# RagnarGrootKoerkamp/astar-pairwise-aligner

Hardware: AMD Instinct MI355X
Metric: DP cell-updates/sec (GCUPS), full bit-parallel DP, 100kbp@5% div (higher is better)
Workload: dtype u32

## Files before the change

astar-pairwise-aligner_amd/csrc/pa_hip.hip:

```cpp
#include "pa_batch.hpp"
#include "engine_capi.hpp"
#include "trace_kernel.hpp"

#include <algorithm>
#include <chrono>
#include <cmath>
#include <cstdio>
#include <cstdlib>
#include <cstring>
#include <memory>
#include <atomic>
#include <mutex>
#include <thread>
#include <string>
#include <vector>

namespace pa {

enum : uint32_t { kTextFailed = 0xFFFFFFFFu };
__global__ __launch_bounds__(64) void format_pack_kernel(const uint32_t* __restrict__ elems, const uint64_t* __restrict__ off,
                                                         const uint32_t* __restrict__ len, const int32_t* __restrict__ list,
                                                         uint8_t* __restrict__ packed, unsigned long long* __restrict__ total,
                                                         uint32_t* __restrict__ tlen, uint64_t* __restrict__ dst) {
    const int pair = list[blockIdx.x];
// ... 674 lines not shown

static pa_batch* batch_create(const BatchInput& in, bool trace, float band_hint = -1.f, int dt_max_g = 0, int dt_fr_drop = 0,
                              const pa_astarpa2_params* astar = nullptr, int window_override = -1) {
    if (!ensure_device()) return nullptr;
    PhaseClock clock("pa_batch_create");
    auto p = std::make_unique<pa_batch>();
    p->pairs = in.pairs;
    p->trace = trace;
    p->dt_max_g = dt_max_g;
    p->dt_fr_drop = dt_fr_drop;
    CreateRun cr{p.get(), in, astar};
    choose_shape(cr, band_hint, window_override);
    if (!layout_pairs(cr) || (trace && !alloc_trace_buffers(cr)) || !alloc_batch_buffers(cr)) return nullptr;
    clock.mark("host layout + hipMalloc");
    if (!(p->stream = bstream_take()) || !hip_ok(hipEventCreate(&p->ev0), "event") ||
        !hip_ok(hipEventCreate(&p->ev1), "event") || !hip_ok(hipEventCreate(&p->ev2), "event"))
        return nullptr;
    clock.mark("stream + events");
    if (!upload_sequences(cr)) return nullptr;
    clock.mark("upload of the sequences");
    std::vector<int32_t> first;
    plan_strip_jobs(cr, first);
    if (!upload_first_and_desc(cr, first)) return nullptr;
    if (trace && in.pairs) {
        std::vector<TraceJob> tjobs(in.pairs);
        std::vector<uint64_t> src_off(in.pairs);
        if (!make_trace_jobs(cr, tjobs, src_off) || !plan_chunks(cr) || !upload_trace_jobs(cr, tjobs, src_off)) return nullptr;
    }
    apply_pacing(p.get());
    if (!attach_wavelog(p.get())) return nullptr;
    clock.mark("jobs + descriptors");
    if (cr.slice_rows) {
        p->sequential = false;
        p->sliced = slice::create(p->n.data(), p->m.data(), in.pairs, p->code_off.data(), p->prof_off.data(), cr.slice_rows);
        if (!p->sliced) return nullptr;
        clock.mark("bit-sliced plan");
    }
    if (!p->d_jobs.alloc(p->jobs.size() * sizeof(StripJob))) return nullptr;
    if (!p->jobs.empty() &&
        !hip_ok(hipMemcpyAsync(p->d_jobs.ptr, p->jobs.data(), p->jobs.size() * sizeof(StripJob), hipMemcpyHostToDevice, p->stream), "H2D jobs"))
        return nullptr;
    if (!hip_ok(hipStreamSynchronize(p->stream), "sync")) return nullptr;
    return p.release();
}

extern "C" pa_batch* pa_batch_create(const uint8_t* const* a, const size_t* a_len, const uint8_t* const* b,
                                     const size_t* b_len, size_t pairs) {
    return batch_create({a, a_len, b, b_len, pairs}, false);
}

extern "C" pa_batch* pa_batch_create_banded(const uint8_t* const* a, const size_t* a_len, const uint8_t* const* b,
                                            const size_t* b_len, size_t pairs, float divergence_hint) {
    if (!(divergence_hint >= 0.f)) {
        set_error("pa_batch_create_banded: divergence_hint must be >= 0");
        return nullptr;
    }
    return batch_create({a, a_len, b, b_len, pairs}, false, divergence_hint);
}

extern "C" pa_batch* pa_batch_create_trace(const uint8_t* const* a, const size_t* a_len, const uint8_t* const* b,
                                           const size_t* b_len, size_t pairs) {
    return batch_create({a, a_len, b, b_len, pairs}, true);
}

extern "C" pa_batch* pa_batch_create_trace_params(const uint8_t* const* a, const size_t* a_len, const uint8_t* const* b,
                                                  const size_t* b_len, size_t pairs, const pa_astarpa2_params* trace_params) {
    if (!trace_params) return batch_create({a, a_len, b, b_len, pairs}, true);
// ... 200 lines not shown
        set_error(timeout_msg, misc[err_word]);
        return PA_E_TIMEOUT;
    }
    return 0;
}

static void dump_wavelog(const pa_batch* p) {
    std::vector<uint32_t> log(p->jobs.size() * 8);
    if (hip_ok(hipMemcpy(log.data(), p->d_wavelog.ptr, log.size() * 4, hipMemcpyDeviceToHost), "D2H wavelog")) {
        if (FILE* f = std::fopen(getenv("PA_STRIP_WAVELOG"), "w")) {
            std::fprintf(f, "job k word0 xcc se cu simd wave t0 t1 polled\n");
            for (size_t j = 0; j < p->jobs.size(); ++j) {
                const uint32_t* r = &log[8 * j];
                const uint32_t hw = r[0];
                std::fprintf(f, "%zu %d %d %u %u %u %u %u %llu %llu %u\n", j, p->sequential ? p->jobs[j].k : p->k, p->jobs[j].word0, r[1] & 15u,
                             (hw >> 13) & 7u, (hw >> 8) & 15u, (hw >> 4) & 3u, hw & 15u, (unsigned long long)(r[2] | ((uint64_t)r[3] << 32)),
                             (unsigned long long)(r[4] | ((uint64_t)r[5] << 32)), r[6]);
            }
            std::fclose(f);
        }
    }
}

extern "C" int pa_batch_run(pa_batch* p, int32_t* cost_out, float* kernel_ms) {
    if (!p) return PA_E_ARG;
    if (p->astar) {
        float fwd = 0.f;
        const int rc = pa_batch_align(p, cost_out, nullptr, &fwd, nullptr);
        if (kernel_ms) *kernel_ms = fwd;
        return rc;
    }
    hipStream_t s = p->stream;
    if (p->sliced) {
        if (const int rc = batch_forward(p, false)) return rc;
        if (const int rc = slice::run(p->sliced, s, p->d_codes.as<uint32_t>(), p->d_prof.as<uint64_t>(), p->d_sums.as<int32_t>(), p->d_misc.as<uint32_t>() + 4,
                                      p->ev0, p->ev1))
            return rc;
        if (const int rc = read_sums_and_errors(p, cost_out, 5, "device spin timeout in the bit-sliced kernel (err=%u)")) return rc;
        if (kernel_ms && !hip_ok(hipEventElapsedTime(kernel_ms, p->ev0, p->ev1), "elapsed")) return PA_E_HIP;
        for (size_t i = 0; i < p->pairs; ++i)
            if (p->n[i] == 0 || p->m[i] == 0) cost_out[i] = (int32_t)(p->n[i] + p->m[i]);
        return 0;
    }
    if (const int rc = batch_forward(p)) return rc;
    std::vector<int32_t> sums(p->pairs, 0);
    if (const int rc = read_sums_and_errors(p, sums.data(), 1, "device spin timeout (err=%u)")) return rc;
    p->gran_dirty = p->banded && !p->sequential;
    if (p->d_wavelog.ptr) dump_wavelog(p);
    if (kernel_ms) {
        *kernel_ms = 0.f;
        if (!p->jobs.empty() && !hip_ok(hipEventElapsedTime(kernel_ms, p->ev0, p->ev1), "elapsed")) return PA_E_HIP;
    }
    if (p->banded) return banded_finish(p, sums, cost_out, kernel_ms);
    for (size_t i = 0; i < p->pairs; ++i) {
        const size_t n = p->n[i], m = p->m[i], w = (m + 63) / 64;
        if (n == 0) { cost_out[i] = (int32_t)m; continue; }
        if (w == 0) { cost_out[i] = (int32_t)n; continue; }
        cost_out[i] = (int32_t)(w * 64) + sums[i];
    }
    return 0;
}

static pa_astarpa2_params traced_batch_params() {
    engine::AstarPa2Params p = engine::AstarPa2Params::nw();
    p.front.sparse = true;
    p.front.dt_trace = false;
    p.front.incremental_doubling = false;
    pa_astarpa2_params c;
    engine::params_to_c(p, &c);
    return c;
}
// ... 541 lines not shown
```

astar-pairwise-aligner_amd/csrc/pa_hip_internal.hpp:

```cpp
#pragma once
#include <hip/hip_runtime.h>

#include <cstddef>
#include <cstdint>
#include <string>
#include <vector>

#include "../../include/pa_astarpa2.h"
#include "../../include/pa_bitpacking_hip.h"
#include "strip_kernel.hpp"

namespace pa {

constexpr int kWordsPerStrip = 32;

void set_error(const char* fmt, ...);
bool hip_ok(hipError_t e, const char* what);
bool ensure_device();
int device_cus();
int fail(int rc, const char* fmt, ...) __attribute__((format(printf, 2, 3)));

void* pinned_take(size_t bytes, size_t* got);
void pinned_give(void* ptr, size_t size);
hipStream_t stream_take();
// ... 64 lines not shown
    int fill_stride = 0, fill_word0 = 0;
    bool pingpong = false;
    int k = 1;
    uint32_t* ckpt = nullptr;
    int ckpt_stride = 0;
};

void plan_rect(std::vector<StripJob>& jobs, const RectPlan& r);
struct StripPlan {
    int full = 0, tail1 = 0;
    int strips() const { return full + tail1; }
};
StripPlan strip_plan(int w, int k, bool sequential);
size_t rect_granules(int n, int w, int k = 1, bool pingpong = false);
bool launch_strips(const StripJob* d_jobs, int njobs, bool fill, uint32_t* d_ticket_err, hipStream_t s, bool zero_ticket = true,
                   bool scatter = false, int k = 1, int block_waves = kStripBlockWaves, bool ckpt = false);
bool launch_pairs(const StripJob* d_jobs, const int32_t* d_first, int npairs, uint32_t* d_ticket_err, hipStream_t s, int k, bool ckpt = false);
int align_hip(const uint8_t* a, size_t a_len, const uint8_t* b, size_t b_len, const pa_astarpa2_params& params, bool trace, bool self_check,
              int32_t* cost_out, std::string* cigar_out, pa_astarpa2_stats* stats_out);
bool combine_eligible(size_t a_len, size_t b_len, const pa_astarpa2_params& params);
struct CombineInside {
    CombineInside();
    ~CombineInside();
    CombineInside(const CombineInside&) = delete;
    CombineInside& operator=(const CombineInside&) = delete;
};
int combine_align(const uint8_t* a, size_t a_len, const uint8_t* b, size_t b_len, const pa_astarpa2_params& params, int32_t* cost_out,
                  std::string* cigar_out, pa_astarpa2_stats* stats_out);
int search_profile(const uint8_t* pattern, size_t plen, float unmatched_cost, std::vector<uint64_t>& prof, std::vector<uint64_t>& v0);
bool encode_a_device(const uint8_t* d_a, int n, uint32_t* d_codes, uint32_t* d_bad, hipStream_t s);
bool build_b_device(const uint8_t* d_b, int m, uint64_t* d_prof, uint32_t* d_bad, hipStream_t s);
bool encode_pair_device(const uint8_t* d_a, int n, uint32_t* d_codes, int code_words, const uint8_t* d_b, int m, uint64_t* d_prof, uint32_t* bad,
                        hipStream_t s);
struct PairDesc {
    unsigned long long a_off, b_off, code_off, prof_off;
    int n, m;
};
bool encode_batch_device(const uint8_t* d_a_cat, size_t max_n, uint32_t* d_codes_cat, const uint8_t* d_b_cat, size_t max_m, uint64_t* d_prof_cat,
                         const PairDesc* d_desc, size_t pairs, uint32_t* d_bad, hipStream_t s);
unsigned host_threads();
size_t window_words(size_t n, size_t m, bool gcsh, int override_);

}
```

astar-pairwise-aligner_amd/csrc/rect_unit.hip:

```cpp
#include "pa_hip_internal.hpp"

#include <algorithm>
#include <cstdlib>
#include <cstring>
#include <mutex>
#include <set>
#include <utility>
#include <vector>

namespace pa {


__device__ __forceinline__ int rank_acgt(uint8_t c) {
    return c == 'A' ? 0 : c == 'C' ? 1 : c == 'G' ? 2 : c == 'T' ? 3 : -1;
}

__global__ void encode_a_kernel(const uint8_t* __restrict__ a, int n, uint32_t* __restrict__ codes, int nwords,
                                uint32_t* __restrict__ bad) {
    const int i = blockIdx.x * blockDim.x + threadIdx.x;
    if (i >= nwords) return;
    uint32_t w = 0;
    bool invalid = false;
    for (int k = 0; k < 16; ++k) {
        const int c = i * 16 + k;
        if (c < n) {
            const int r = rank_acgt(a[c]);
            invalid |= r < 0;
            w |= (uint32_t)(r & 3) << (2 * k);
        }
    }
    codes[i] = w;
    if (invalid) atomicOr(bad, 1u);
}

__global__ void build_b_kernel(const uint8_t* __restrict__ b, int m, uint64_t* __restrict__ prof, int nwords,
                               uint32_t* __restrict__ bad) {
    const int word = blockIdx.x * (blockDim.x >> 6) + (threadIdx.x >> 6);
    if (word >= nwords) return;
    const int lane = threadIdx.x & 63;
    const int j = word * 64 + lane;
    int r = 3;
    bool invalid = false;
    if (j < m) {
        r = rank_acgt(b[j]);
        invalid = r < 0;
        r &= 3;
    }
    const uint64_t nb0 = __ballot(((r & 1) ^ 1) != 0);
// ... 451 lines not shown
```

astar-pairwise-aligner_amd/csrc/slice_kernel.hpp:

```cpp
#pragma once
#include <hip/hip_runtime.h>
#include <stdint.h>

namespace pa {
namespace slice {

#ifndef PA_SLICE_CLOCK_TURNS
#define PA_SLICE_CLOCK_TURNS 15
#endif
#ifndef PA_SLICE_YIELD
#define PA_SLICE_YIELD 2
#endif
constexpr int kPad = 64;
constexpr int kErrSpin = 7;
constexpr uint32_t kSpinLimit = 1u << 22;

struct SliceGroup {
    uint64_t a_off;
    uint64_t b_off;
    uint64_t h_off;
    uint32_t h_stride;
    int32_t n;
    int32_t nstrips;
    int32_t npairs;
    uint32_t first_pos;
    uint32_t ev_first, ev_count;
    uint32_t pad_;
};
struct SliceEvent {
    int32_t col;
    uint32_t mask;
};
struct SliceJob {
    uint32_t group, strip;
};
struct SlicePair {
    uint64_t code_off, prof_off;
    int32_t n, m;
    uint32_t pair;
    uint32_t pad_;
};

typedef uint32_t pa_slice_u32x2 __attribute__((ext_vector_type(2)));
__device__ __forceinline__ uint32_t dpp_wave_shr1(uint32_t old_, uint32_t src) {
    return (uint32_t)__builtin_amdgcn_update_dpp((int)old_, (int)src, 0x138, 0xf, 0xf, false);
}
__device__ __forceinline__ uint32_t dpp_wave_rol1(uint32_t x) {
    return (uint32_t)__builtin_amdgcn_update_dpp((int)x, (int)x, 0x134, 0xf, 0xf, false);
}
__device__ __forceinline__ uint2 ld_boundary(const uint2* p) {
    const unsigned long long v = __hip_atomic_load((const unsigned long long*)p, __ATOMIC_RELAXED, __HIP_MEMORY_SCOPE_AGENT);
    return make_uint2((uint32_t)v, (uint32_t)(v >> 32));
}
__device__ __forceinline__ void st_boundary(uint2* p, uint32_t hp, uint32_t hm) {
    __hip_atomic_store((unsigned long long*)p, (unsigned long long)hp | ((unsigned long long)hm << 32), __ATOMIC_RELAXED, __HIP_MEMORY_SCOPE_AGENT);
}

#define PA_SLICE_ROW_PAIR(vpA, vmA, vpB, vmB, nb0A, nb1A, nb0B, nb1B, a0, a1, hpp, hmp, hpo, hmo)                                      \
    do {                                                                                                                                \
        uint32_t zA_, zB_, hmA_, hpA_;                                                                                                  \
        asm volatile(                                                                                                                   \
            "v_xor_b32 %[zA], %[a1_], %[nb1A_]\n\t"                                                                                     \
            "v_xor_b32 %[zB], %[a1_], %[nb1B_]\n\t"                                                                                     \
            "v_bitop3_b32 %[zA], %[a0_], %[nb0A_], %[zA] bitop3:0x28\n\t"                                                               \
            "v_bitop3_b32 %[zB], %[a0_], %[nb0B_], %[zB] bitop3:0x28\n\t"                                                               \
            "v_bitop3_b32 %[zA], %[zA], %[vmA_], %[hmp_] bitop3:0xfe\n\t"                                                               \
            "v_and_b32 %[hmA], %[zA], %[vpA_]\n\t"                                                                                      \
            "v_bitop3_b32 %[hpA], %[vmA_], %[zA], %[vpA_] bitop3:0xf1\n\t"                                                              \
            "v_bitop3_b32 %[zB], %[zB], %[vmB_], %[hmA] bitop3:0xfe\n\t"                                                                \
            "v_bitop3_b32 %[vpA_], %[hmp_], %[zA], %[hpp_] bitop3:0xf1\n\t"                                                             \
            "v_and_b32 %[hmB], %[zB], %[vpB_]\n\t"                                                                                      \
            "v_and_b32 %[vmA_], %[hpp_], %[zA]\n\t"                                                                                     \
            "v_bitop3_b32 %[hpB], %[vmB_], %[zB], %[vpB_] bitop3:0xf1\n\t"                                                              \
            "v_bitop3_b32 %[vpB_], %[hmA], %[zB], %[hpA] bitop3:0xf1\n\t"                                                               \
            "v_and_b32 %[vmB_], %[hpA], %[zB]"                                                                                          \
            : [zA] "=&v"(zA_), [zB] "=&v"(zB_), [hmA] "=&v"(hmA_), [hpA] "=&v"(hpA_), [hmB] "=&v"(hmo), [hpB] "=&v"(hpo),              \
              [vpA_] "+v"(vpA), [vmA_] "+v"(vmA), [vpB_] "+v"(vpB), [vmB_] "+v"(vmB)                                                    \
            : [a0_] "v"(a0), [a1_] "v"(a1), [nb0A_] "v"(nb0A), [nb1A_] "v"(nb1A), [nb0B_] "v"(nb0B), [nb1B_] "v"(nb1B), [hpp_] "v"(hpp), \
              [hmp_] "v"(hmp));                                                                                                         \
    } while (0)

#define PA_SLICE_FEED(a0, a1, hpp, hmp, ohp, ohm, cAx, cAy, cHx, cHy)                                                                    \
    asm volatile(                                                                                                                       \
        "s_mov_b64 vcc, 1\n\t"                                                                                                          \
        "v_cndmask_b32_dpp %[a0_], %[a0_], %[cAx_], vcc wave_shr:1 row_mask:0xf bank_mask:0xf bound_ctrl:0\n\t"                         \
        "v_cndmask_b32_dpp %[a1_], %[a1_], %[cAy_], vcc wave_shr:1 row_mask:0xf bank_mask:0xf bound_ctrl:0\n\t"                         \
        "v_cndmask_b32_dpp %[hpp_], %[ohp_], %[cHx_], vcc wave_shr:1 row_mask:0xf bank_mask:0xf bound_ctrl:0\n\t"                       \
        "v_cndmask_b32_dpp %[hmp_], %[ohm_], %[cHy_], vcc wave_shr:1 row_mask:0xf bank_mask:0xf bound_ctrl:0\n\t"                       \
        "v_mov_b32_dpp %[cAx_], %[cAx_] wave_rol:1 row_mask:0xf bank_mask:0xf\n\t"                                                      \
        "v_mov_b32_dpp %[cAy_], %[cAy_] wave_rol:1 row_mask:0xf bank_mask:0xf\n\t"                                                      \
        "v_mov_b32_dpp %[cHx_], %[cHx_] wave_rol:1 row_mask:0xf bank_mask:0xf\n\t"                                                      \
        "v_mov_b32_dpp %[cHy_], %[cHy_] wave_rol:1 row_mask:0xf bank_mask:0xf"                                                          \
        : [a0_] "+v"(a0), [a1_] "+v"(a1), [hpp_] "=&v"(hpp), [hmp_] "=&v"(hmp), [cAx_] "+v"(cAx), [cAy_] "+v"(cAy), [cHx_] "+v"(cHx),   \
          [cHy_] "+v"(cHy)                                                                                                              \
        : [ohp_] "v"(ohp), [ohm_] "v"(ohm)                                                                                              \
        : "vcc")

template <int R>
__global__ __launch_bounds__(64, 2) void slice_kernel(const SliceJob* __restrict__ jobs, int njobs, const SliceGroup* __restrict__ groups,
                                                      const SliceEvent* __restrict__ events, const uint2* __restrict__ A, const uint2* __restrict__ B,
                                                      uint2* H, uint2* V, uint32_t* ticket_err, unsigned long long* dbg) {
    static_assert(R % 2 == 0, "rows are stepped in pairs");
    const int lane = (int)threadIdx.x;
    const uint32_t wave_slot = (uint32_t)__builtin_amdgcn_s_getreg((4 - 1) << 11 | 4) & 15u;
    for (;;) {
        uint32_t tk = 0;
        if (lane == 0) tk = atomicAdd(ticket_err, 1u);
        tk = (uint32_t)__builtin_amdgcn_readfirstlane((int)tk);
        if (tk >= (uint32_t)njobs) break;
        const SliceJob job = jobs[tk];
        const SliceGroup grp = groups[job.group];
        const unsigned long long t_job0 = dbg ? __builtin_amdgcn_s_memrealtime() : 0ull;
        unsigned long long t_parked = 0, n_parks = 0;
        [[maybe_unused]] bool waited_before = false;
        [[maybe_unused]] int slack = 0;
        const int s = (int)job.strip, n = grp.n;
        const bool has_in = s > 0, has_out = s + 1 < grp.nstrips;
        const uint2* Ag = A + grp.a_off + kPad;
        const size_t row0 = grp.b_off + ((size_t)s * 64 + (size_t)lane) * R;
        const uint2* Hin = H + grp.h_off + (size_t)(has_in ? s - 1 : 0) * grp.h_stride + kPad;
        uint2* Hout = H + grp.h_off + (size_t)(has_out ? s : 0) * grp.h_stride + kPad;
        const SliceEvent* ev = events + grp.ev_first;
        uint32_t nb0[R], nb1[R], vp[R], vm[R];
#pragma unroll
        for (int i = 0; i < R; ++i) {
            const uint2 b = B[row0 + i];
            nb0[i] = b.x;
            nb1[i] = b.y;
            vp[i] = ~0u;
            vm[i] = 0u;
        }
        constexpr int kWaitStep = 8;
        uint32_t a0 = 0, a1 = 0, o_hp = 0, o_hm = ~0u;
        uint32_t off = (lane == 63 && has_out) ? (uint32_t)(-lane) * 8u : 0x7FFFFFF0u;
        int cnt = 1 - lane;
// ... 11 lines not shown
            if ((((uint32_t)__builtin_amdgcn_s_memrealtime() >> PA_SLICE_CLOCK_TURNS) ^ wave_slot) & 1u) __builtin_amdgcn_s_setprio(1);
            else __builtin_amdgcn_s_setprio(0);
#else
            if (((uint32_t)q ^ wave_slot) & 1u) __builtin_amdgcn_s_setprio(1);
            else __builtin_amdgcn_s_setprio(0);
#endif
            uint2 cA = kA, cH = kH;
            const int col = q * 64 + lane;
            if (has_in) {
                uint32_t spins = 0;
                const unsigned long long t_p0 = dbg ? __builtin_amdgcn_s_memrealtime() : 0ull;
                while (col < n && (cH.x & cH.y) != 0u) {
                    __builtin_amdgcn_s_sleep(32);
                    cH = ld_boundary(Hin + col);
                    if (++spins > kSpinLimit) {
                        atomicCAS(ticket_err + 1, 0u, (uint32_t)kErrSpin);
                        cH = make_uint2(~0u, 0u);
                    }
                }
                const bool waited = __builtin_amdgcn_readfirstlane((int)(__ballot(spins != 0u) != 0ull)) != 0;
#if PA_SLICE_YIELD == 1
                if (waited) __builtin_amdgcn_s_setprio(0);
#elif PA_SLICE_YIELD == 2
                if (waited || waited_before) __builtin_amdgcn_s_setprio(0);
                waited_before = waited;
#elif PA_SLICE_YIELD >= 3
                slack = waited ? PA_SLICE_YIELD : (slack > 0 ? slack - 1 : 0);
                if (slack > 0) __builtin_amdgcn_s_setprio(0);
#endif
                if (dbg && waited) {
                    t_parked += __builtin_amdgcn_s_memrealtime() - t_p0;
                    n_parks += 1;
                }
            }
            const int pcol = min(col + 64, n + kPad - 1);
            const bool more = q + 1 < nchunks;
            if (more) {
                asm volatile("global_load_dwordx2 %0, %1, off ; pa_prefetch_load" : "=v"(nA) : "v"(Ag + pcol) : "memory");
                if (has_in) asm volatile("global_load_dwordx2 %0, %1, off sc1 ; pa_prefetch_load" : "=v"(nH) : "v"(Hin + pcol) : "memory");
            }
            const int jend = min(64, n + 63 - q * 64);
            const int wait_at = more ? kWaitStep : -1;
            for (int j = 0; j < jend; ++j) {
                asm volatile("" : "+s"(j));
                if (j == wait_at) {
                    asm volatile("s_waitcnt vmcnt(8) ; pa_prefetch_wait" : "+v"(nA), "+v"(nH)::"memory");
                    kA = make_uint2((uint32_t)nA, (uint32_t)(nA >> 32));
                    if (has_in) kH = make_uint2((uint32_t)nH, (uint32_t)(nH >> 32));
                }
                uint32_t hpp, hmp;
                PA_SLICE_FEED(a0, a1, hpp, hmp, o_hp, o_hm, cA.x, cA.y, cH.x, cH.y);
#pragma unroll
                for (int i = 0; i < R; i += 2) {
                    uint32_t hpo, hmo;
                    PA_SLICE_ROW_PAIR(vp[i], vm[i], vp[i + 1], vm[i + 1], nb0[i], nb1[i], nb0[i + 1], nb1[i + 1], a0, a1, hpp, hmp, hpo, hmo);
                    hpp = hpo;
                    hmp = hmo;
                }
                o_hp = hpp;
                o_hm = hmp;
                {
                    const pa_slice_u32x2 d = {hpp, hmp};
                    __builtin_amdgcn_raw_buffer_store_b64(d, hrs, off, 0, 16);
                }
                off += 8u;
                if (cnt == ev_col) {
                    const uint32_t mask = ev[ev_i].mask;
#pragma unroll
                    for (int i = 0; i < R; ++i) {
                        atomicOr(&V[row0 + i].x, vp[i] & mask);
                        atomicOr(&V[row0 + i].y, vm[i] & mask);
                        asm volatile("" ::: "memory");
                    }
                    ++ev_i;
                    ev_col = ev_i < grp.ev_count ? ev[ev_i].col : kNoEvent;
                    __builtin_amdgcn_s_waitcnt(0);
                }
                ++cnt;
            }
        }
        if (dbg && lane == 0) {
            const unsigned long long dt = __builtin_amdgcn_s_memrealtime() - t_job0;
            atomicMin(dbg + 0, dt);
            atomicMax(dbg + 1, dt);
            atomicAdd(dbg + 2, dt);
            atomicAdd(dbg + 3, 1ull);
            atomicAdd(dbg + 4, t_parked);
            atomicAdd(dbg + 5, n_parks);
            if (s == 0) {
                atomicMin(dbg + 6, dt);
                atomicMax(dbg + 7, dt);
            }
            const uint32_t xcc = (uint32_t)__builtin_amdgcn_s_getreg((4 - 1) << 11 | 20) & 7u;
            atomicAdd(dbg + 8 + 2 * xcc, dt - t_parked);
            atomicAdd(dbg + 9 + 2 * xcc, 1ull);
        }
    }
}


__global__ __launch_bounds__(256) void slice_pack_a_kernel(const SliceGroup* __restrict__ groups, const SlicePair* __restrict__ spairs,
                                                           const uint32_t* __restrict__ codes, uint2* __restrict__ A) {
    const SliceGroup grp = groups[blockIdx.x];
    const int lane = (int)(threadIdx.x & 63), q = (int)(blockIdx.y * 4 + (threadIdx.x >> 6));
    if (q * 32 >= grp.n) return;
    const int p = lane & 31, half = lane >> 5, word = 2 * q + half;
    uint32_t w = 0;
    if (p < grp.npairs) {
        const SlicePair sp = spairs[grp.first_pos + p];
        if (word < (sp.n + 15) / 16) w = codes[sp.code_off + word];
    }
    uint32_t a0 = 0, a1 = 0;
#pragma unroll
    for (int k = 0; k < 16; ++k) {
        const unsigned long long b0 = __ballot((w >> (2 * k)) & 1u), b1 = __ballot((w >> (2 * k + 1)) & 1u);
        if ((lane & 15) == k) {
            a0 = (lane & 16) ? (uint32_t)(b0 >> 32) : (uint32_t)b0;
            a1 = (lane & 16) ? (uint32_t)(b1 >> 32) : (uint32_t)b1;
        }
    }
    const int c = q * 32 + lane;
    if (lane < 32 && c < grp.n) A[grp.a_off + kPad + c] = make_uint2(a0, a1);
}

__global__ __launch_bounds__(256) void slice_pack_b_kernel(const SliceGroup* __restrict__ groups, const SlicePair* __restrict__ spairs,
                                                           const uint64_t* __restrict__ prof, uint2* __restrict__ B, int rows_per_strip) {
    const SliceGroup grp = groups[blockIdx.x];
    const int lane = (int)(threadIdx.x & 63), j = (int)(blockIdx.y * 4 + (threadIdx.x >> 6));
    if ((long long)j * 64 >= (long long)grp.nstrips * rows_per_strip) return;
    const int p = lane & 31, half = lane >> 5;
    uint32_t x0 = 0, x1 = 0;
    if (p < grp.npairs) {
        const SlicePair sp = spairs[grp.first_pos + p];
        if (j < (sp.m + 63) / 64) {
            const uint64_t p0 = prof[2 * (sp.prof_off + j)], p1 = prof[2 * (sp.prof_off + j) + 1];
            x0 = (uint32_t)(p0 >> (32 * half));
            x1 = (uint32_t)(p1 >> (32 * half));
        }
    }
    uint32_t nb0 = 0, nb1 = 0;
#pragma unroll
    for (int k = 0; k < 32; ++k) {
        const unsigned long long b0 = __ballot((x0 >> k) & 1u), b1 = __ballot((x1 >> k) & 1u);
        if ((lane & 31) == k) {
            nb0 = half ? (uint32_t)(b0 >> 32) : (uint32_t)b0;
            nb1 = half ? (uint32_t)(b1 >> 32) : (uint32_t)b1;
        }
    }
    B[grp.b_off + (size_t)j * 64 + lane] = make_uint2(nb0, nb1);
}

constexpr int kScoreSpan = 4096;
__global__ __launch_bounds__(64) void slice_score_kernel(const SliceGroup* __restrict__ groups, const SlicePair* __restrict__ spairs,
                                                         const uint2* __restrict__ V, int32_t* __restrict__ cost_out) {
    const SliceGroup grp = groups[blockIdx.x];
    const int lane = (int)threadIdx.x;
    int my_m = 0, my_n = 0;
    uint32_t my_pair = 0;
    if (lane < grp.npairs) {
        const SlicePair sp = spairs[grp.first_pos + lane];
        my_m = sp.m;
        my_n = sp.n;
        my_pair = sp.pair;
    }
    int max_m = my_m;
#pragma unroll
    for (int o = 32; o > 0; o >>= 1) max_m = max(max_m, __shfl_xor(max_m, o));
    const int lo = (int)blockIdx.y * kScoreSpan, hi = min(max_m, lo + kScoreSpan);
    if (lo >= max_m) return;
    int acc = blockIdx.y == 0 ? my_n : 0;
    for (int r0 = lo; r0 < hi; r0 += 64) {
        const int r = r0 + lane;
// ... 15 lines not shown
```

astar-pairwise-aligner_amd/csrc/slice_plan.hpp:

```cpp
#pragma once
#include <hip/hip_runtime.h>

#include <cstddef>
#include <cstdint>

namespace pa {
namespace slice {

struct Plan;

constexpr int kRowsPerLane[] = {52, 50, 48, 46, 44, 42, 40, 36, 32, 28};

int choose_rows_per_lane(const size_t* a_len, const size_t* b_len, size_t pairs, double simds, double* est_ns);

Plan* create(const size_t* a_len, const size_t* b_len, size_t pairs, const size_t* code_off, const size_t* prof_off, int rows_per_lane);
void destroy(Plan* p);

int run(Plan* p, hipStream_t s, const uint32_t* d_codes, const uint64_t* d_prof, int32_t* d_costs, uint32_t* d_ticket_err, hipEvent_t ev0, hipEvent_t ev1);

struct Info {
    int rows_per_lane;
    size_t groups, jobs;
    double valu_instructions;
    double computed_rows_cells;
    double device_bytes;
    double boundary_bytes;
};
Info info(const Plan* p);
constexpr int kStepOverheadInstr = 11;

}
}
```

astar-pairwise-aligner_amd/csrc/slice_unit.hip:

```cpp
#include "slice_plan.hpp"

#include <algorithm>
#include <cmath>
#include <cstdio>
#include <cstdlib>
#include <memory>
#include <numeric>
#include <vector>

#include "pa_hip_internal.hpp"
#include "slice_kernel.hpp"

namespace pa {
namespace slice {

struct Plan {
    int R = 52;
    size_t pairs = 0;
    std::vector<SliceGroup> groups;
    std::vector<SliceJob> jobs;
    size_t a_elems = 0, b_elems = 0, h_elems = 0;
    unsigned max_col_blocks = 0, max_row_blocks = 0;
    double valu = 0, computed = 0;
    DeviceBuf d_groups, d_events, d_jobs, d_spairs, d_A, d_B, d_V, d_H;
};

static int strips_for(size_t m, int R) { return (int)((m + (size_t)64 * R - 1) / ((size_t)64 * R)); }

static constexpr double kNsPerRowStep = 16.2, kNsStepOverhead = 25.6, kChainPenalty = 0.0015;

int choose_rows_per_lane(const size_t* a_len, const size_t* b_len, size_t pairs, double simds, double* est_ns) {
    if (const char* e = getenv("PA_SLICE")) {
        if (atoi(e) == 0) return 0;
    }
    size_t live = 0;
    for (size_t i = 0; i < pairs; ++i) {
        live += a_len[i] > 0 && b_len[i] > 0;
        if (a_len[i] >= (size_t(1) << 27) || b_len[i] >= (size_t(1) << 27)) return 0;
    }
    const bool forced = getenv("PA_SLICE") && atoi(getenv("PA_SLICE")) > 0;
    if (live < 64 && !forced) return 0;
    std::vector<uint32_t> order;
    for (size_t i = 0; i < pairs; ++i)
        if (a_len[i] > 0 && b_len[i] > 0) order.push_back((uint32_t)i);
    std::sort(order.begin(), order.end(), [&](uint32_t x, uint32_t y) { return a_len[x] != a_len[y] ? a_len[x] < a_len[y] : (b_len[x] != b_len[y] ? b_len[x] < b_len[y] : x < y); });
    int best_r = 0;
    double best = -1;
    const double slots = simds * 2.0;
    for (const int R : kRowsPerLane) {
        if (forced && atoi(getenv("PA_SLICE")) > 1 && atoi(getenv("PA_SLICE")) != R) continue;
        double work = 0, longest = 0, jobs = 0;
        for (size_t g = 0; g * 32 < order.size(); ++g) {
            size_t n = 0, m = 0;
            for (size_t t = g * 32; t < std::min(order.size(), g * 32 + 32); ++t) {
                n = std::max(n, a_len[order[t]]);
                m = std::max(m, b_len[order[t]]);
            }
            const int S = strips_for(m, R);
            const double per_strip = ((double)n + 63.0) * (R * kNsPerRowStep + kNsStepOverhead) * (1.0 + kChainPenalty * (S - 1));
            work += per_strip * S;
            jobs += S;
            longest = std::max(longest, per_strip + 128.0 * (S - 1) * (R * kNsPerRowStep + kNsStepOverhead));
        }
        const double waves = std::min(jobs, slots);
        const double speed = waves <= simds ? 1.165 : 1.0 + 0.165 * (slots - waves) / simds;
        const double rounds = jobs > slots ? std::ceil(jobs / slots) * (work / jobs) : work / waves;
        const double t = std::max(longest / 1.165, rounds / speed);
        if (best < 0 || t < best) {
            best = t;
            best_r = R;
        }
    }
    if (est_ns) *est_ns = best;
    return best_r;
}

Plan* create(const size_t* a_len, const size_t* b_len, size_t pairs, const size_t* code_off, const size_t* prof_off, int rows_per_lane) {
    auto p = std::make_unique<Plan>();
    p->R = rows_per_lane;
    p->pairs = pairs;
    const int R = rows_per_lane;
    std::vector<uint32_t> order;
    for (size_t i = 0; i < pairs; ++i)
        if (a_len[i] > 0 && b_len[i] > 0) order.push_back((uint32_t)i);
    std::sort(order.begin(), order.end(), [&](uint32_t x, uint32_t y) { return a_len[x] != a_len[y] ? a_len[x] < a_len[y] : (b_len[x] != b_len[y] ? b_len[x] < b_len[y] : x < y); });
    std::vector<SlicePair> spairs(order.size());
    std::vector<SliceEvent> events;
    size_t a_at = 0, b_at = 0, h_at = 0;
    size_t max_n = 0, max_rows = 0;
    const size_t ngroups = (order.size() + 31) / 32;
    for (size_t gi = 0; gi < ngroups; ++gi) {
        const size_t g = ngroups - 1 - gi;
        SliceGroup grp{};
        grp.first_pos = (uint32_t)(g * 32);
        grp.npairs = (int32_t)std::min<size_t>(32, order.size() - g * 32);
        size_t n = 0, m = 0;
        for (int t = 0; t < grp.npairs; ++t) {
            const uint32_t i = order[g * 32 + t];
            n = std::max(n, a_len[i]);
            m = std::max(m, b_len[i]);
            spairs[g * 32 + t] = SlicePair{(uint64_t)code_off[i], (uint64_t)prof_off[i], (int32_t)a_len[i], (int32_t)b_len[i], i, 0u};
        }
        grp.n = (int32_t)n;
        grp.nstrips = strips_for(m, R);
        grp.a_off = a_at;
        grp.b_off = b_at;
        grp.h_off = h_at;
        grp.h_stride = (uint32_t)(n + 2 * kPad);
        a_at += n + 2 * kPad;
        b_at += (size_t)grp.nstrips * 64 * R;
        h_at += (size_t)(grp.nstrips - 1) * grp.h_stride;
        grp.ev_first = (uint32_t)events.size();
        for (int t = 0; t < grp.npairs; ++t) {
            const int32_t col = (int32_t)a_len[order[g * 32 + t]];
            if (events.size() > grp.ev_first && events.back().col == col) events.back().mask |= 1u << t;
            else events.push_back(SliceEvent{col, 1u << t});
        }
        grp.ev_count = (uint32_t)events.size() - grp.ev_first;
        max_n = std::max(max_n, n);
        max_rows = std::max(max_rows, (size_t)grp.nstrips * 64 * R);
        for (int s = 0; s < grp.nstrips; ++s) p->jobs.push_back(SliceJob{(uint32_t)p->groups.size(), (uint32_t)s});
        p->valu += (double)grp.nstrips * ((double)n + 63.0) * (7.0 * R + kStepOverheadInstr);
        p->computed += (double)grp.nstrips * 64.0 * R * (double)n * 32.0;
        p->groups.push_back(grp);
    }
    p->a_elems = a_at;
    p->b_elems = b_at;
    p->h_elems = h_at;
    p->max_col_blocks = (unsigned)((max_n + 127) / 128);
    p->max_row_blocks = (unsigned)((max_rows / 64 + 3) / 4);
    if (p->groups.empty()) return p.release();
    if (events.empty()) events.push_back(SliceEvent{0, 0});
    if (!p->d_groups.alloc(p->groups.size() * sizeof(SliceGroup)) || !p->d_events.alloc(events.size() * sizeof(SliceEvent)) ||
        !p->d_jobs.alloc(p->jobs.size() * sizeof(SliceJob)) || !p->d_spairs.alloc(spairs.size() * sizeof(SlicePair)) || !p->d_A.alloc(a_at * 8) ||
        !p->d_B.alloc(b_at * 8) || !p->d_V.alloc(b_at * 8) || !p->d_H.alloc(std::max<size_t>(h_at, 8) * 8))
        return nullptr;
    if (!hip_ok(hipMemcpy(p->d_groups.ptr, p->groups.data(), p->groups.size() * sizeof(SliceGroup), hipMemcpyHostToDevice), "H2D slice groups") ||
        !hip_ok(hipMemcpy(p->d_events.ptr, events.data(), events.size() * sizeof(SliceEvent), hipMemcpyHostToDevice), "H2D slice events") ||
        !hip_ok(hipMemcpy(p->d_jobs.ptr, p->jobs.data(), p->jobs.size() * sizeof(SliceJob), hipMemcpyHostToDevice), "H2D slice jobs") ||
        !hip_ok(hipMemcpy(p->d_spairs.ptr, spairs.data(), spairs.size() * sizeof(SlicePair), hipMemcpyHostToDevice), "H2D slice pairs") ||
        !hip_ok(hipMemset(p->d_A.ptr, 0, a_at * 8), "memset slice A"))
        return nullptr;
    return p.release();
}

void destroy(Plan* p) { delete p; }

template <int R>
static hipError_t launch_slice(int grid, hipStream_t s, const Plan* p, uint32_t* d_ticket_err, unsigned long long* dbg) {
    hipLaunchKernelGGL((slice_kernel<R>), dim3((unsigned)grid), dim3(64), 0, s, p->d_jobs.as<SliceJob>(), (int)p->jobs.size(), p->d_groups.as<SliceGroup>(),
                       p->d_events.as<SliceEvent>(), p->d_A.as<uint2>(), p->d_B.as<uint2>(), p->d_H.as<uint2>(), p->d_V.as<uint2>(), d_ticket_err, dbg);
    return hipGetLastError();
}

int run(Plan* p, hipStream_t s, const uint32_t* d_codes, const uint64_t* d_prof, int32_t* d_costs, uint32_t* d_ticket_err, hipEvent_t ev0, hipEvent_t ev1) {
    if (!hip_ok(hipMemsetAsync(d_ticket_err, 0, 8, s), "memset slice ticket")) return PA_E_HIP;
    if (p->groups.empty()) {
        if (ev0 && (!hip_ok(hipEventRecord(ev0, s), "event") || !hip_ok(hipEventRecord(ev1, s), "event"))) return PA_E_HIP;
        return 0;
    }
    const unsigned G = (unsigned)p->groups.size();
    hipLaunchKernelGGL(slice_pack_a_kernel, dim3(G, p->max_col_blocks), dim3(256), 0, s, p->d_groups.as<SliceGroup>(), p->d_spairs.as<SlicePair>(), d_codes,
                       p->d_A.as<uint2>());
    hipLaunchKernelGGL(slice_pack_b_kernel, dim3(G, p->max_row_blocks), dim3(256), 0, s, p->d_groups.as<SliceGroup>(), p->d_spairs.as<SlicePair>(), d_prof,
                       p->d_B.as<uint2>(), 64 * p->R);
    if (!hip_ok(hipGetLastError(), "slice transposes")) return PA_E_HIP;
    if (!hip_ok(hipMemsetAsync(p->d_V.ptr, 0, p->b_elems * 8, s), "memset slice V")) return PA_E_HIP;
    if (p->h_elems && !hip_ok(hipMemsetAsync(p->d_H.ptr, 0xFF, p->h_elems * 8, s), "memset slice boundaries")) return PA_E_HIP;
    const int grid = (int)std::min<size_t>(p->jobs.size(), (size_t)device_cus() * 8);
    static const bool jobtimes = getenv("PA_SLICE_JOBTIMES") != nullptr;
    unsigned long long* dbg = nullptr;
    if (jobtimes && hipMalloc((void**)&dbg, 192) == hipSuccess) {
        const unsigned long long init[24] = {~0ull, 0, 0, 0, 0, 0, ~0ull, 0};
        if (hipMemcpyAsync(dbg, init, 192, hipMemcpyHostToDevice, s) != hipSuccess || hipStreamSynchronize(s) != hipSuccess) dbg = nullptr;
    }
    if (ev0 && !hip_ok(hipEventRecord(ev0, s), "event")) return PA_E_HIP;
    hipError_t e = hipSuccess;
    switch (p->R) {
        case 52: e = launch_slice<52>(grid, s, p, d_ticket_err, dbg); break;
        case 50: e = launch_slice<50>(grid, s, p, d_ticket_err, dbg); break;
        case 48: e = launch_slice<48>(grid, s, p, d_ticket_err, dbg); break;
        case 46: e = launch_slice<46>(grid, s, p, d_ticket_err, dbg); break;
        case 44: e = launch_slice<44>(grid, s, p, d_ticket_err, dbg); break;
        case 42: e = launch_slice<42>(grid, s, p, d_ticket_err, dbg); break;
        case 40: e = launch_slice<40>(grid, s, p, d_ticket_err, dbg); break;
        case 36: e = launch_slice<36>(grid, s, p, d_ticket_err, dbg); break;
        case 32: e = launch_slice<32>(grid, s, p, d_ticket_err, dbg); break;
        case 28: e = launch_slice<28>(grid, s, p, d_ticket_err, dbg); break;
        default: set_error("slice: no kernel for %d rows per lane", p->R); return PA_E_INTERNAL;
    }
    if (!hip_ok(e, "slice_kernel")) return PA_E_HIP;
    if (ev1 && !hip_ok(hipEventRecord(ev1, s), "event")) return PA_E_HIP;
    if (dbg) {
        unsigned long long h[24] = {0};
        if (hipMemcpyAsync(h, dbg, 192, hipMemcpyDeviceToHost, s) == hipSuccess && hipStreamSynchronize(s) == hipSuccess && h[3]) {
            std::fprintf(stderr, "[slice jobs] awake us per job by XCD:");
            for (int x = 0; x < 8; ++x) std::fprintf(stderr, " %d: %.0f (%llu)", x, h[9 + 2 * x] ? h[8 + 2 * x] * 0.01 / (double)h[9 + 2 * x] : 0.0, h[9 + 2 * x]);
            std::fprintf(stderr, "\n");
            std::fprintf(stderr, "[slice jobs] R %d: %llu jobs, us per job: min %.1f mean %.1f max %.1f (first strips: min %.1f max %.1f); asleep behind the strip above: %.2f %% of the job time, %.1f waits per job\n",
                         p->R, h[3], h[0] * 0.01, h[2] * 0.01 / (double)h[3], h[1] * 0.01, h[6] * 0.01, h[7] * 0.01, 100.0 * (double)h[4] / (double)h[2], (double)h[5] / (double)h[3]);
        }
        (void)hipFree(dbg);
    }
    hipLaunchKernelGGL(slice_score_kernel, dim3(G, (p->max_row_blocks * 256u + kScoreSpan - 1) / kScoreSpan), dim3(64), 0, s, p->d_groups.as<SliceGroup>(), p->d_spairs.as<SlicePair>(), p->d_V.as<uint2>(), d_costs);
    if (!hip_ok(hipGetLastError(), "slice_score_kernel")) return PA_E_HIP;
    return 0;
}

Info info(const Plan* p) {
    Info i{};
    i.rows_per_lane = p->R;
    i.groups = p->groups.size();
    i.jobs = p->jobs.size();
    i.valu_instructions = p->valu;
    i.computed_rows_cells = p->computed;
// ... 8 lines not shown
```

Baseline: 243,900.

## Pack bit-sliced inputs directly from raw sequences and allow odd rows per lane

The bit-sliced path no longer runs the batch forward encoding pass that produced 2-bit codes and profiles. The slice pack kernels now read the raw ACGT bytes directly, rank them, and flag invalid characters. The kernel resets its boundary cells as it consumes them, so the full H memset is skipped on clean reruns. Odd rows-per-lane values (45, 47, 49, 51) are added through a single-row step, which gives the rows-per-lane chooser finer choices. The cost is more complex pack kernels with unaligned uint4 reads, and a dirty-flag protocol that has to stay correct across error paths.

```diff
diff --git a/astar-pairwise-aligner_amd/csrc/pa_hip.hip b/astar-pairwise-aligner_amd/csrc/pa_hip.hip
--- a/astar-pairwise-aligner_amd/csrc/pa_hip.hip
+++ b/astar-pairwise-aligner_amd/csrc/pa_hip.hip
@@ -730,7 +730,7 @@
     clock.mark("jobs + descriptors");
     if (cr.slice_rows) {
         p->sequential = false;
-        p->sliced = slice::create(p->n.data(), p->m.data(), in.pairs, p->code_off.data(), p->prof_off.data(), cr.slice_rows);
+        p->sliced = slice::create(p->n.data(), p->m.data(), in.pairs, p->a_off.data(), p->b_off.data(), cr.slice_rows);
         if (!p->sliced) return nullptr;
         clock.mark("bit-sliced plan");
     }
@@ -997,11 +997,14 @@
     }
     hipStream_t s = p->stream;
     if (p->sliced) {
-        if (const int rc = batch_forward(p, false)) return rc;
-        if (const int rc = slice::run(p->sliced, s, p->d_codes.as<uint32_t>(), p->d_prof.as<uint64_t>(), p->d_sums.as<int32_t>(), p->d_misc.as<uint32_t>() + 4,
-                                      p->ev0, p->ev1))
+        if (!hip_ok(hipMemsetAsync(p->d_misc.ptr, 0, 32, s), "memset") ||
+            !hip_ok(hipMemsetAsync(p->d_sums.ptr, 0, std::max<size_t>(p->pairs * 4, 16), s), "memset sums"))
+            return PA_E_HIP;
+        if (const int rc = slice::run(p->sliced, s, p->d_a.as<uint8_t>(), p->d_b.as<uint8_t>(), p->d_misc.as<uint32_t>() + 3, p->d_sums.as<int32_t>(),
+                                      p->d_misc.as<uint32_t>() + 4, p->ev0, p->ev1))
             return rc;
         if (const int rc = read_sums_and_errors(p, cost_out, 5, "device spin timeout in the bit-sliced kernel (err=%u)")) return rc;
+        slice::mark_clean(p->sliced);
         if (kernel_ms && !hip_ok(hipEventElapsedTime(kernel_ms, p->ev0, p->ev1), "elapsed")) return PA_E_HIP;
         for (size_t i = 0; i < p->pairs; ++i)
             if (p->n[i] == 0 || p->m[i] == 0) cost_out[i] = (int32_t)(p->n[i] + p->m[i]);
diff --git a/astar-pairwise-aligner_amd/csrc/pa_hip_internal.hpp b/astar-pairwise-aligner_amd/csrc/pa_hip_internal.hpp
--- a/astar-pairwise-aligner_amd/csrc/pa_hip_internal.hpp
+++ b/astar-pairwise-aligner_amd/csrc/pa_hip_internal.hpp
@@ -120,6 +120,10 @@
 bool build_b_device(const uint8_t* d_b, int m, uint64_t* d_prof, uint32_t* d_bad, hipStream_t s);
 bool encode_pair_device(const uint8_t* d_a, int n, uint32_t* d_codes, int code_words, const uint8_t* d_b, int m, uint64_t* d_prof, uint32_t* bad,
                         hipStream_t s);
+__device__ __forceinline__ int rank_acgt(uint8_t c) {
+    return c == 'A' ? 0 : c == 'C' ? 1 : c == 'G' ? 2 : c == 'T' ? 3 : -1;
+}
+
 struct PairDesc {
     unsigned long long a_off, b_off, code_off, prof_off;
     int n, m;
diff --git a/astar-pairwise-aligner_amd/csrc/rect_unit.hip b/astar-pairwise-aligner_amd/csrc/rect_unit.hip
--- a/astar-pairwise-aligner_amd/csrc/rect_unit.hip
+++ b/astar-pairwise-aligner_amd/csrc/rect_unit.hip
@@ -10,10 +10,6 @@
 
 namespace pa {
 
-
-__device__ __forceinline__ int rank_acgt(uint8_t c) {
-    return c == 'A' ? 0 : c == 'C' ? 1 : c == 'G' ? 2 : c == 'T' ? 3 : -1;
-}
 
 __global__ void encode_a_kernel(const uint8_t* __restrict__ a, int n, uint32_t* __restrict__ codes, int nwords,
                                 uint32_t* __restrict__ bad) {
diff --git a/astar-pairwise-aligner_amd/csrc/slice_kernel.hpp b/astar-pairwise-aligner_amd/csrc/slice_kernel.hpp
--- a/astar-pairwise-aligner_amd/csrc/slice_kernel.hpp
+++ b/astar-pairwise-aligner_amd/csrc/slice_kernel.hpp
@@ -35,7 +35,7 @@
     uint32_t group, strip;
 };
 struct SlicePair {
-    uint64_t code_off, prof_off;
+    uint64_t a_off, b_off;
     int32_t n, m;
     uint32_t pair;
     uint32_t pad_;
@@ -80,6 +80,21 @@
               [hmp_] "v"(hmp));                                                                                                         \
     } while (0)
 
+#define PA_SLICE_ROW_ONE(vpA, vmA, nb0A, nb1A, a0, a1, hpp, hmp, hpo, hmo)                                                              \
+    do {                                                                                                                                \
+        uint32_t zA_;                                                                                                                   \
+        asm volatile(                                                                                                                   \
+            "v_xor_b32 %[zA], %[a1_], %[nb1A_]\n\t"                                                                                     \
+            "v_bitop3_b32 %[zA], %[a0_], %[nb0A_], %[zA] bitop3:0x28\n\t"                                                               \
+            "v_bitop3_b32 %[zA], %[zA], %[vmA_], %[hmp_] bitop3:0xfe\n\t"                                                               \
+            "v_and_b32 %[hmA], %[zA], %[vpA_]\n\t"                                                                                      \
+            "v_bitop3_b32 %[hpA], %[vmA_], %[zA], %[vpA_] bitop3:0xf1\n\t"                                                              \
+            "v_bitop3_b32 %[vpA_], %[hmp_], %[zA], %[hpp_] bitop3:0xf1\n\t"                                                             \
+            "v_and_b32 %[vmA_], %[hpp_], %[zA]"                                                                                          \
+            : [zA] "=&v"(zA_), [hmA] "=&v"(hmo), [hpA] "=&v"(hpo), [vpA_] "+v"(vpA), [vmA_] "+v"(vmA)                                   \
+            : [a0_] "v"(a0), [a1_] "v"(a1), [nb0A_] "v"(nb0A), [nb1A_] "v"(nb1A), [hpp_] "v"(hpp), [hmp_] "v"(hmp));                    \
+    } while (0)
+
 #define PA_SLICE_FEED(a0, a1, hpp, hmp, ohp, ohm, cAx, cAy, cHx, cHy)                                                                    \
     asm volatile(                                                                                                                       \
         "s_mov_b64 vcc, 1\n\t"                                                                                                          \
@@ -100,7 +115,6 @@
 __global__ __launch_bounds__(64, 2) void slice_kernel(const SliceJob* __restrict__ jobs, int njobs, const SliceGroup* __restrict__ groups,
                                                       const SliceEvent* __restrict__ events, const uint2* __restrict__ A, const uint2* __restrict__ B,
                                                       uint2* H, uint2* V, uint32_t* ticket_err, unsigned long long* dbg) {
-    static_assert(R % 2 == 0, "rows are stepped in pairs");
     const int lane = (int)threadIdx.x;
     const uint32_t wave_slot = (uint32_t)__builtin_amdgcn_s_getreg((4 - 1) << 11 | 4) & 15u;
     for (;;) {
@@ -178,6 +192,7 @@
                     t_parked += __builtin_amdgcn_s_memrealtime() - t_p0;
                     n_parks += 1;
                 }
+                if (col < n) st_boundary(const_cast<uint2*>(Hin) + col, ~0u, ~0u);
             }
             const int pcol = min(col + 64, n + kPad - 1);
             const bool more = q + 1 < nchunks;
@@ -197,9 +212,15 @@
                 uint32_t hpp, hmp;
                 PA_SLICE_FEED(a0, a1, hpp, hmp, o_hp, o_hm, cA.x, cA.y, cH.x, cH.y);
 #pragma unroll
-                for (int i = 0; i < R; i += 2) {
+                for (int i = 0; i + 1 < R; i += 2) {
                     uint32_t hpo, hmo;
                     PA_SLICE_ROW_PAIR(vp[i], vm[i], vp[i + 1], vm[i + 1], nb0[i], nb1[i], nb0[i + 1], nb1[i + 1], a0, a1, hpp, hmp, hpo, hmo);
+                    hpp = hpo;
+                    hmp = hmo;
+                }
+                if constexpr (R & 1) {
+                    uint32_t hpo, hmo;
+                    PA_SLICE_ROW_ONE(vp[R - 1], vm[R - 1], nb0[R - 1], nb1[R - 1], a0, a1, hpp, hmp, hpo, hmo);
                     hpp = hpo;
                     hmp = hmo;
                 }
@@ -245,17 +266,33 @@
 }
 
 
+__device__ __forceinline__ uint32_t slice_rank16(const uint4 v, int count, bool& invalid) {
+    const uint32_t q[4] = {v.x, v.y, v.z, v.w};
+    uint32_t w = 0;
+#pragma unroll
+    for (int k = 0; k < 16; ++k) {
+        const int r = rank_acgt((uint8_t)(q[k >> 2] >> (8 * (k & 3))));
+        if (k < count) {
+            invalid |= r < 0;
+            w |= (uint32_t)(r & 3) << (2 * k);
+        }
+    }
+    return w;
+}
+
 __global__ __launch_bounds__(256) void slice_pack_a_kernel(const SliceGroup* __restrict__ groups, const SlicePair* __restrict__ spairs,
-                                                           const uint32_t* __restrict__ codes, uint2* __restrict__ A) {
-    const SliceGroup grp = groups[blockIdx.x];
-    const int lane = (int)(threadIdx.x & 63), q = (int)(blockIdx.y * 4 + (threadIdx.x >> 6));
-    if (q * 32 >= grp.n) return;
-    const int p = lane & 31, half = lane >> 5, word = 2 * q + half;
+                                                           const uint8_t* __restrict__ a_cat, uint2* __restrict__ A, uint32_t* __restrict__ bad) {
+    const SliceGroup grp = groups[blockIdx.y];
+    const int lane = (int)(threadIdx.x & 63), q = (int)(blockIdx.x * 4 + (threadIdx.x >> 6));
+    if ((long long)q * 32 >= (long long)grp.n) return;
+    const int p = lane & 31, half = lane >> 5, c0 = 32 * q + 16 * half;
     uint32_t w = 0;
+    bool invalid = false;
     if (p < grp.npairs) {
         const SlicePair sp = spairs[grp.first_pos + p];
-        if (word < (sp.n + 15) / 16) w = codes[sp.code_off + word];
-    }
+        if (c0 < sp.n) w = slice_rank16(*(const uint4*)(a_cat + sp.a_off + c0), sp.n - c0, invalid);
+    }
+    if (invalid) atomicOr(bad, 1u);
     uint32_t a0 = 0, a1 = 0;
 #pragma unroll
     for (int k = 0; k < 16; ++k) {
@@ -270,20 +307,36 @@
 }
 
 __global__ __launch_bounds__(256) void slice_pack_b_kernel(const SliceGroup* __restrict__ groups, const SlicePair* __restrict__ spairs,
-                                                           const uint64_t* __restrict__ prof, uint2* __restrict__ B, int rows_per_strip) {
-    const SliceGroup grp = groups[blockIdx.x];
-    const int lane = (int)(threadIdx.x & 63), j = (int)(blockIdx.y * 4 + (threadIdx.x >> 6));
+                                                           const uint8_t* __restrict__ b_cat, uint2* __restrict__ B, int rows_per_strip,
+                                                           uint32_t* __restrict__ bad) {
+    const SliceGroup grp = groups[blockIdx.y];
+    const int lane = (int)(threadIdx.x & 63), j = (int)(blockIdx.x * 4 + (threadIdx.x >> 6));
     if ((long long)j * 64 >= (long long)grp.nstrips * rows_per_strip) return;
     const int p = lane & 31, half = lane >> 5;
+    const long long r0 = (long long)j * 64 + 32 * half;
     uint32_t x0 = 0, x1 = 0;
+    bool invalid = false;
     if (p < grp.npairs) {
         const SlicePair sp = spairs[grp.first_pos + p];
-        if (j < (sp.m + 63) / 64) {
-            const uint64_t p0 = prof[2 * (sp.prof_off + j)], p1 = prof[2 * (sp.prof_off + j) + 1];
-            x0 = (uint32_t)(p0 >> (32 * half));
-            x1 = (uint32_t)(p1 >> (32 * half));
-        }
-    }
+#pragma unroll
+        for (int h = 0; h < 2; ++h) {
+            const long long r = r0 + 16 * h;
+            if (r < (long long)sp.m) {
+                const int count = (int)min((long long)sp.m - r, 16ll);
+                const uint32_t w = slice_rank16(*(const uint4*)(b_cat + sp.b_off + r), count, invalid);
+                const uint32_t real = count >= 16 ? ~0u : (1u << (2 * count)) - 1u, nw = ~w & real;
+                uint32_t e = 0, o = 0;
+#pragma unroll
+                for (int k = 0; k < 16; ++k) {
+                    e |= ((nw >> (2 * k)) & 1u) << k;
+                    o |= ((nw >> (2 * k + 1)) & 1u) << k;
+                }
+                x0 |= e << (16 * h);
+                x1 |= o << (16 * h);
+            }
+        }
+    }
+    if (invalid) atomicOr(bad, 1u);
     uint32_t nb0 = 0, nb1 = 0;
 #pragma unroll
     for (int k = 0; k < 32; ++k) {
diff --git a/astar-pairwise-aligner_amd/csrc/slice_plan.hpp b/astar-pairwise-aligner_amd/csrc/slice_plan.hpp
--- a/astar-pairwise-aligner_amd/csrc/slice_plan.hpp
+++ b/astar-pairwise-aligner_amd/csrc/slice_plan.hpp
@@ -9,14 +9,16 @@
 
 struct Plan;
 
-constexpr int kRowsPerLane[] = {52, 50, 48, 46, 44, 42, 40, 36, 32, 28};
+constexpr int kRowsPerLane[] = {52, 51, 50, 49, 48, 47, 46, 45, 44, 42, 40, 36, 32, 28};
 
 int choose_rows_per_lane(const size_t* a_len, const size_t* b_len, size_t pairs, double simds, double* est_ns);
 
-Plan* create(const size_t* a_len, const size_t* b_len, size_t pairs, const size_t* code_off, const size_t* prof_off, int rows_per_lane);
+Plan* create(const size_t* a_len, const size_t* b_len, size_t pairs, const size_t* a_off, const size_t* b_off, int rows_per_lane);
 void destroy(Plan* p);
 
-int run(Plan* p, hipStream_t s, const uint32_t* d_codes, const uint64_t* d_prof, int32_t* d_costs, uint32_t* d_ticket_err, hipEvent_t ev0, hipEvent_t ev1);
+int run(Plan* p, hipStream_t s, const uint8_t* d_a, const uint8_t* d_b, uint32_t* d_bad, int32_t* d_costs, uint32_t* d_ticket_err, hipEvent_t ev0,
+        hipEvent_t ev1);
+void mark_clean(Plan* p);
 
 struct Info {
     int rows_per_lane;
diff --git a/astar-pairwise-aligner_amd/csrc/slice_unit.hip b/astar-pairwise-aligner_amd/csrc/slice_unit.hip
--- a/astar-pairwise-aligner_amd/csrc/slice_unit.hip
+++ b/astar-pairwise-aligner_amd/csrc/slice_unit.hip
@@ -22,6 +22,7 @@
     size_t a_elems = 0, b_elems = 0, h_elems = 0;
     unsigned max_col_blocks = 0, max_row_blocks = 0;
     double valu = 0, computed = 0;
+    bool h_dirty = false;
     DeviceBuf d_groups, d_events, d_jobs, d_spairs, d_A, d_B, d_V, d_H;
 };
 
@@ -39,6 +40,7 @@
         if (a_len[i] >= (size_t(1) << 27) || b_len[i] >= (size_t(1) << 27)) return 0;
     }
     const bool forced = getenv("PA_SLICE") && atoi(getenv("PA_SLICE")) > 0;
+    if ((live + 31) / 32 > 65535) return 0;
     if (live < 64 && !forced) return 0;
     std::vector<uint32_t> order;
     for (size_t i = 0; i < pairs; ++i)
@@ -75,7 +77,7 @@
     return best_r;
 }
 
-Plan* create(const size_t* a_len, const size_t* b_len, size_t pairs, const size_t* code_off, const size_t* prof_off, int rows_per_lane) {
+Plan* create(const size_t* a_len, const size_t* b_len, size_t pairs, const size_t* a_off, const size_t* b_off, int rows_per_lane) {
     auto p = std::make_unique<Plan>();
     p->R = rows_per_lane;
     p->pairs = pairs;
@@ -99,7 +101,7 @@
             const uint32_t i = order[g * 32 + t];
             n = std::max(n, a_len[i]);
             m = std::max(m, b_len[i]);
-            spairs[g * 32 + t] = SlicePair{(uint64_t)code_off[i], (uint64_t)prof_off[i], (int32_t)a_len[i], (int32_t)b_len[i], i, 0u};
+            spairs[g * 32 + t] = SlicePair{(uint64_t)a_off[i], (uint64_t)b_off[i], (int32_t)a_len[i], (int32_t)b_len[i], i, 0u};
         }
         grp.n = (int32_t)n;
         grp.nstrips = strips_for(m, R);
@@ -139,12 +141,15 @@
         !hip_ok(hipMemcpy(p->d_events.ptr, events.data(), events.size() * sizeof(SliceEvent), hipMemcpyHostToDevice), "H2D slice events") ||
         !hip_ok(hipMemcpy(p->d_jobs.ptr, p->jobs.data(), p->jobs.size() * sizeof(SliceJob), hipMemcpyHostToDevice), "H2D slice jobs") ||
         !hip_ok(hipMemcpy(p->d_spairs.ptr, spairs.data(), spairs.size() * sizeof(SlicePair), hipMemcpyHostToDevice), "H2D slice pairs") ||
-        !hip_ok(hipMemset(p->d_A.ptr, 0, a_at * 8), "memset slice A"))
+        !hip_ok(hipMemset(p->d_A.ptr, 0, a_at * 8), "memset slice A") ||
+        (h_at && !hip_ok(hipMemset(p->d_H.ptr, 0xFF, h_at * 8), "memset slice boundaries")))
         return nullptr;
     return p.release();
 }
 
 void destroy(Plan* p) { delete p; }
+
+void mark_clean(Plan* p) { p->h_dirty = false; }
 
 template <int R>
 static hipError_t launch_slice(int grid, hipStream_t s, const Plan* p, uint32_t* d_ticket_err, unsigned long long* dbg) {
@@ -153,20 +158,22 @@
     return hipGetLastError();
 }
 
-int run(Plan* p, hipStream_t s, const uint32_t* d_codes, const uint64_t* d_prof, int32_t* d_costs, uint32_t* d_ticket_err, hipEvent_t ev0, hipEvent_t ev1) {
+int run(Plan* p, hipStream_t s, const uint8_t* d_a, const uint8_t* d_b, uint32_t* d_bad, int32_t* d_costs, uint32_t* d_ticket_err, hipEvent_t ev0,
+        hipEvent_t ev1) {
     if (!hip_ok(hipMemsetAsync(d_ticket_err, 0, 8, s), "memset slice ticket")) return PA_E_HIP;
     if (p->groups.empty()) {
         if (ev0 && (!hip_ok(hipEventRecord(ev0, s), "event") || !hip_ok(hipEventRecord(ev1, s), "event"))) return PA_E_HIP;
         return 0;
     }
     const unsigned G = (unsigned)p->groups.size();
-    hipLaunchKernelGGL(slice_pack_a_kernel, dim3(G, p->max_col_blocks), dim3(256), 0, s, p->d_groups.as<SliceGroup>(), p->d_spairs.as<SlicePair>(), d_codes,
-                       p->d_A.as<uint2>());
-    hipLaunchKernelGGL(slice_pack_b_kernel, dim3(G, p->max_row_blocks), dim3(256), 0, s, p->d_groups.as<SliceGroup>(), p->d_spairs.as<SlicePair>(), d_prof,
-                       p->d_B.as<uint2>(), 64 * p->R);
+    hipLaunchKernelGGL(slice_pack_a_kernel, dim3(p->max_col_blocks, G), dim3(256), 0, s, p->d_groups.as<SliceGroup>(), p->d_spairs.as<SlicePair>(), d_a,
+                       p->d_A.as<uint2>(), d_bad);
+    hipLaunchKernelGGL(slice_pack_b_kernel, dim3(p->max_row_blocks, G), dim3(256), 0, s, p->d_groups.as<SliceGroup>(), p->d_spairs.as<SlicePair>(), d_b,
+                       p->d_B.as<uint2>(), 64 * p->R, d_bad);
     if (!hip_ok(hipGetLastError(), "slice transposes")) return PA_E_HIP;
     if (!hip_ok(hipMemsetAsync(p->d_V.ptr, 0, p->b_elems * 8, s), "memset slice V")) return PA_E_HIP;
-    if (p->h_elems && !hip_ok(hipMemsetAsync(p->d_H.ptr, 0xFF, p->h_elems * 8, s), "memset slice boundaries")) return PA_E_HIP;
+    if (p->h_elems && p->h_dirty && !hip_ok(hipMemsetAsync(p->d_H.ptr, 0xFF, p->h_elems * 8, s), "memset slice boundaries")) return PA_E_HIP;
+    p->h_dirty = true;
     const int grid = (int)std::min<size_t>(p->jobs.size(), (size_t)device_cus() * 8);
     static const bool jobtimes = getenv("PA_SLICE_JOBTIMES") != nullptr;
     unsigned long long* dbg = nullptr;
@@ -178,9 +185,13 @@
     hipError_t e = hipSuccess;
     switch (p->R) {
         case 52: e = launch_slice<52>(grid, s, p, d_ticket_err, dbg); break;
+        case 51: e = launch_slice<51>(grid, s, p, d_ticket_err, dbg); break;
         case 50: e = launch_slice<50>(grid, s, p, d_ticket_err, dbg); break;
+        case 49: e = launch_slice<49>(grid, s, p, d_ticket_err, dbg); break;
         case 48: e = launch_slice<48>(grid, s, p, d_ticket_err, dbg); break;
+        case 47: e = launch_slice<47>(grid, s, p, d_ticket_err, dbg); break;
         case 46: e = launch_slice<46>(grid, s, p, d_ticket_err, dbg); break;
+        case 45: e = launch_slice<45>(grid, s, p, d_ticket_err, dbg); break;
         case 44: e = launch_slice<44>(grid, s, p, d_ticket_err, dbg); break;
         case 42: e = launch_slice<42>(grid, s, p, d_ticket_err, dbg); break;
         case 40: e = launch_slice<40>(grid, s, p, d_ticket_err, dbg); break;
```

After: 254,000 (median of 6 runs). +4.1%, better.
